# KevinMathewT/multimodal-propaganda-meme-classification

Hardware: AMD Instinct MI355X
Metric: memes/sec (fine-tune step) ViT-B/16+BERT-base bs=32, 1/2/4/8 MI355X (higher is better)
Workload: dtype fp16

## Files before the change

include/memehip.h:

```cpp
#ifndef MEMEHIP_H
#define MEMEHIP_H

#include <stdint.h>

#ifdef __cplusplus
extern "C" {
#endif

typedef enum MhStatus {
    MH_OK = 0,
    MH_EINVAL = 1,
    MH_ESHAPE = 2,
    MH_ELAUNCH = 3
} MhStatus;

typedef void* mh_stream_t;

const char* mh_version(void);
const char* mh_status_str(int status);

#define MH_GEMM_MAX_GROUP 8
#define MH_GEMM_GELU 1
#define MH_GEMM_OUT_F32 2
#define MH_GEMM_ACCUM 4
#define MH_GEMM_QUICK_GELU 8
#define MH_GEMM_DERIV_AUX 16

typedef struct MhGemmProblem {
    const void* A;
    const void* B;
    void* C;
    const float* bias;
    const void* residual;
    void* aux;
    const void* mul;
    float* rowsum;
    int32_t M, N, K;
    int32_t lda, ldb, ldc;
    int32_t flags;
    float alpha;
    const uint32_t* drop_rng;
    float drop_p;
    uint32_t drop_stream;
    const int32_t* rows_dev;
    const int32_t* drop_rows;
    int32_t ksplit;
    int32_t reserved_;
} MhGemmProblem;

int mh_gemm_bf16_grouped(const MhGemmProblem* problems , int n_problems, int a_kmajor,
                         int b_kmajor, mh_stream_t stream);
int mh_gemm_ksplit_for(int K, int want);
int mh_gemm_set_trace(void* device_buffer);

int mh_layernorm_fwd(const void* x , const float* gamma, const float* beta, void* y ,
                     float* y_f32 , float* mean, float* rstd,
                     int rows, int D, float eps, mh_stream_t stream);
int mh_layernorm_bwd(const void* dy , const void* x , const float* gamma,
                     const float* mean, const float* rstd, const void* dx_add ,
                     void* dx , float* part , int n_part, int rows, int D,
                     void* dx_drop ,
                     const uint32_t* rng, float drop_p, uint32_t drop_stream, mh_stream_t stream);
#define MH_LN_MAX_JOBS 4
typedef struct MhLnFwdJob {
    const void* x; const float* gamma; const float* beta; void* y; float* y_f32; float* mean; float* rstd;
    int32_t rows; float eps;
    const int32_t* rows_dev;
} MhLnFwdJob;
typedef struct MhLnBwdJob {
    const void* dy; const void* x; const float* gamma; const float* mean; const float* rstd;
    const void* dx_add; void* dx; float* part; void* dx_drop; const uint32_t* rng;
    int32_t n_part; int32_t rows; float drop_p; uint32_t drop_stream;
    const int32_t* rows_dev;
    const int32_t* drop_rows;
} MhLnBwdJob;
int mh_layernorm_fwd_grouped(const MhLnFwdJob* jobs, int n_jobs, int D, mh_stream_t stream);
int mh_layernorm_bwd_grouped(const MhLnBwdJob* jobs, int n_jobs, int D, mh_stream_t stream);
#define MH_COLSUM_MAX_JOBS 64
typedef struct MhColsumJob {
    const float* part;
    float* out0;
    float* out1;
} MhColsumJob;
int mh_colsum_partials_f32(const MhColsumJob* jobs , int n_jobs, int n_part, int D,
                           float scale, mh_stream_t stream);

int mh_attn_fwd(const void* qkv, const int64_t* key_mask, void* out, float* lse, int B, int S, int H,
                const uint32_t* rng, float drop_p, uint32_t drop_stream, mh_stream_t stream);
int mh_attn_bwd(const void* qkv, const int64_t* key_mask, const void* out, const void* dout,
                const float* lse, float* delta, void* dqkv, int B, int S, int H, const uint32_t* rng,
                float drop_p, uint32_t drop_stream, mh_stream_t stream);
int mh_attn_fwd_packed(const void* qkv, const int64_t* key_mask, void* out, float* lse, const int32_t* cu,
                       const int32_t* row_map, int B, int S, int H, const uint32_t* rng, float drop_p,
                       uint32_t drop_stream, mh_stream_t stream);
int mh_attn_bwd_packed(const void* qkv, const int64_t* key_mask, const void* out, const void* dout,
                       const float* lse, float* delta, void* dqkv, const int32_t* cu, const int32_t* row_map, int B,
                       int S, int H, const uint32_t* rng, float drop_p, uint32_t drop_stream, mh_stream_t stream);

#define MH_ATTN_MAX_GROUP 2
typedef struct MhAttnProblem {
    const void* qkv; const int64_t* key_mask; void* out; float* lse;
    const void* dout; float* delta; void* dqkv;
    const int32_t* cu; const int32_t* row_map;
    const uint32_t* rng; float drop_p; uint32_t drop_stream;
    int32_t B, S, H; int32_t reserved;
} MhAttnProblem;
int mh_attn_fwd_grouped(const MhAttnProblem* problems , int n, mh_stream_t stream);
int mh_attn_bwd_grouped(const MhAttnProblem* problems , int n, mh_stream_t stream);
int mh_attn_set_onepass(int on);

int mh_pack_plan(const int64_t* mask , int B, int S, int pool_index, int32_t* cu, int32_t* row_map,
                 int32_t* inv_map, int64_t* pmask, int32_t* pool_rows, int32_t* n_rows, mh_stream_t stream);
int mh_pack_rows(const void* src , const int32_t* row_map, const int32_t* n_rows, void* dst,
                 int max_rows, int D, mh_stream_t stream);
int mh_unpack_rows(const void* src , const int32_t* inv_map, void* dst ,
                   int max_rows, int D, mh_stream_t stream);

#define MH_ROWS_MAX_JOBS 8
typedef struct {
    const void* src;
    void* dst;
    const int32_t* idx;
    const int32_t* rows_dev;
    int32_t n, rows, D, stride, offset; int32_t reserved_;
} MhRowsJob;
int mh_rows_gather(const MhRowsJob* jobs , int n_jobs, mh_stream_t stream);
int mh_rows_scatter_zero(const MhRowsJob* jobs , int n_jobs, mh_stream_t stream);

int mh_bert_embed_fwd(const int64_t* ids, const float* word, const float* pos, const float* type0,
                      const float* gamma, const float* beta, void* pre ,
                      void* y , float* mean, float* rstd, int B, int S, int D, int vocab,
                      float eps, const uint32_t* rng, float drop_p, uint32_t drop_stream ,
                      mh_stream_t stream);
int mh_bert_embed_bwd(const int64_t* ids, const void* d_pre , float* dword ,
                      float* dpos , float* dtype0 , int B, int S, int D,
// ... 251 lines not shown
```

multimodal_propaganda_meme_classification_amd/_lib.py:

```python
from __future__ import annotations

import ctypes as C
import os

_HERE = os.path.dirname(os.path.abspath(__file__))
LIB_PATH = os.path.join(_HERE, "libmemehip.so")
LIB_PATH_F16 = os.path.join(_HERE, "libmemehip_f16.so")
LIB_PATHS = {"bf16": LIB_PATH, "fp16": LIB_PATH_F16}

MH_GEMM_MAX_GROUP = 8
MH_GEMM_GELU = 1
MH_GEMM_OUT_F32 = 2
MH_GEMM_ACCUM = 4
MH_GEMM_QUICK_GELU = 8
MH_GEMM_DERIV_AUX = 16
MH_COLSUM_MAX_JOBS = 64
MH_LN_MAX_JOBS = 4
MH_ATTN_MAX_GROUP = 2

c_void_p, c_int, c_int64, c_float = C.c_void_p, C.c_int, C.c_int64, C.c_float


class MhGemmProblem(C.Structure):
    _fields_ = [("A", c_void_p), ("B", c_void_p), ("C", c_void_p), ("bias", c_void_p),
# ... 17 lines not shown
    _fields_ = [("slabs", c_void_p), ("g", c_void_p)] + [(n, C.c_int32) for n in ("Cout", "Cin", "KH", "KW", "Cp", "ldk", "nsplit", "accumulate")] + \
               [("scale", C.c_float), ("block_start", C.c_int32)]


class MhConvGeom(C.Structure):
    _fields_ = [(n, C.c_int32) for n in ("B", "H", "W", "C", "KH", "KW", "stride", "pad", "Cout", "ldk")]


class MhConvBnBwd(C.Structure):
    _fields_ = [(n, c_void_p) for n in ("z", "mean", "rstd", "gamma", "beta", "part")] + [("relu", C.c_int32), ("reserved_", C.c_int32),
                                                                                          ("addend", c_void_p), ("y_mask", c_void_p)]


class MhConvWgradProblem(C.Structure):
    _fields_ = [("dy", c_void_p), ("x", c_void_p), ("slabs", c_void_p), ("ksplit", C.c_int32), ("alpha", C.c_float), ("geom", MhConvGeom)]


MH_CONV_MAX_GROUP = 6
MH_CONV_MAX_JOBS = 64
MH_BN_RELU, MH_BN_ACCUM_PARAM_GRADS = 1, 2


MH_ADAM_MAX_GROUPS = 8


class MhAdamSkipGroups(C.Structure):
    _fields_ = [("hyper", c_void_p * MH_ADAM_MAX_GROUPS), ("beta1", C.c_double * MH_ADAM_MAX_GROUPS), ("beta2", C.c_double * MH_ADAM_MAX_GROUPS),
                ("n", C.c_int32), ("reserved_", C.c_int32)]


class MhLossScale(C.Structure):
    _fields_ = [("scale", c_void_p), ("growth", c_void_p), ("overflow", c_void_p), ("growth_factor", C.c_float), ("backoff_factor", C.c_float),
                ("min_scale", C.c_float), ("max_scale", C.c_float), ("growth_interval", C.c_int32), ("base_grad_scale", C.c_float)]


class MhLnFwdJob(C.Structure):
    _fields_ = [(n, c_void_p) for n in ("x", "gamma", "beta", "y", "y_f32", "mean", "rstd")] + \
               [("rows", C.c_int32), ("eps", C.c_float), ("rows_dev", c_void_p)]


class MhLnBwdJob(C.Structure):
    _fields_ = [(n, c_void_p) for n in ("dy", "x", "gamma", "mean", "rstd", "dx_add", "dx", "part", "dx_drop", "rng")] + \
               [("n_part", C.c_int32), ("rows", C.c_int32), ("drop_p", C.c_float), ("drop_stream", C.c_uint32),
                ("rows_dev", c_void_p), ("drop_rows", c_void_p)]


class MhAttnProblem(C.Structure):
    _fields_ = [(n, c_void_p) for n in ("qkv", "key_mask", "out", "lse", "dout", "delta", "dqkv", "cu", "row_map", "rng")] + \
               [("drop_p", C.c_float), ("drop_stream", C.c_uint32), ("B", C.c_int32), ("S", C.c_int32), ("H", C.c_int32),
                ("reserved", C.c_int32)]


MH_ROWS_MAX_JOBS = 8


class MhRowsJob(C.Structure):
    _fields_ = [(n, c_void_p) for n in ("src", "dst", "idx", "rows_dev")] + \
               [(n, C.c_int32) for n in ("n", "rows", "D", "stride", "offset", "reserved_")]


class MhGemmF32(C.Structure):
    _fields_ = [("A", c_void_p), ("B", c_void_p), ("C", c_void_p), ("bias", c_void_p)] + \
               [(n, C.c_int32) for n in ("M", "N", "K", "lda", "ldb", "ldc", "flags")] + \
               [(n, c_void_p) for n in ("bn_gamma", "bn_beta", "bn_running_mean", "bn_running_var", "bn_save_mean",
                                        "bn_save_rstd", "bn_z")] + \
               [("bn_ldz", C.c_int32), ("bn_eps", C.c_float), ("bn_momentum", C.c_float), ("bn_training", C.c_int32)]


MH_F32_ACCUM, MH_F32_TANH, MH_F32_RELU, MH_F32_BN = 1, 2, 4, 8


class MhHeadParams(C.Structure):
    _fields_ = [(n, c_void_p) for n in ("Wt", "bt", "Wi", "bi", "Wf", "bf_", "Wo", "bo")]


class MhHeadGrads(C.Structure):
    _fields_ = [(n, c_void_p) for n in ("Wt", "bt", "Wi", "bi", "Wf", "bf_", "Wo", "bo")]


_PROTOS = {
    "mh_gemm_bf16_grouped": [C.POINTER(MhGemmProblem), c_int, c_int, c_int, c_void_p],
    "mh_gemm_set_trace": [c_void_p],
    "mh_gemm_ksplit_for": [c_int, c_int],
    "mh_layernorm_fwd": [c_void_p] * 7 + [c_int, c_int, c_float, c_void_p],
    "mh_layernorm_bwd": [c_void_p] * 8 + [c_int, c_int, c_int, c_void_p, c_void_p, c_float, C.c_uint32, c_void_p],
    "mh_layernorm_fwd_grouped": [C.POINTER(MhLnFwdJob), c_int, c_int, c_void_p],
    "mh_layernorm_bwd_grouped": [C.POINTER(MhLnBwdJob), c_int, c_int, c_void_p],
    "mh_colsum_partials_f32": [C.POINTER(MhColsumJob), c_int, c_int, c_int, c_float, c_void_p],
    "mh_attn_fwd": [c_void_p] * 4 + [c_int, c_int, c_int, c_void_p, c_float, C.c_uint32, c_void_p],
    "mh_attn_bwd": [c_void_p] * 7 + [c_int, c_int, c_int, c_void_p, c_float, C.c_uint32, c_void_p],
    "mh_attn_fwd_grouped": [C.POINTER(MhAttnProblem), c_int, c_void_p],
    "mh_attn_bwd_grouped": [C.POINTER(MhAttnProblem), c_int, c_void_p],
    "mh_attn_set_onepass": [c_int],
    "mh_attn_fwd_packed": [c_void_p] * 6 + [c_int, c_int, c_int, c_void_p, c_float, C.c_uint32, c_void_p],
    "mh_attn_bwd_packed": [c_void_p] * 9 + [c_int, c_int, c_int, c_void_p, c_float, C.c_uint32, c_void_p],
    "mh_pack_plan": [c_void_p, c_int, c_int, c_int] + [c_void_p] * 6 + [c_void_p],
    "mh_pack_rows": [c_void_p] * 4 + [c_int, c_int, c_void_p],
    "mh_unpack_rows": [c_void_p] * 3 + [c_int, c_int, c_void_p],
    "mh_rows_gather": [C.POINTER(MhRowsJob), c_int, c_void_p],
    "mh_rows_scatter_zero": [C.POINTER(MhRowsJob), c_int, c_void_p],
    "mh_bert_embed_fwd": [c_void_p] * 10 + [c_int, c_int, c_int, c_int, c_float, c_void_p, c_float, C.c_uint32, c_void_p],
    "mh_image_normalize_u8": [c_void_p, c_void_p, c_int, c_int, c_int, C.POINTER(c_float), C.POINTER(c_float), c_void_p],
    "mh_image_resample_u8": [c_void_p] * 5 + [c_int] + [c_void_p] * 2 + [c_int] + [c_void_p] * 4 + [c_int] * 5 + [c_void_p],
    "mh_image_luma_sum_u8": [c_void_p, c_void_p, c_int, c_int, c_void_p],
    "mh_image_jitter_rotate_u8": [c_void_p] * 5 + [c_int] * 3 + [c_void_p],
    "mh_dropout_apply": [c_void_p, c_int64, c_void_p, c_float, C.c_uint32, c_void_p],
    "mh_dropout_mask_u8": [c_void_p, c_int64, c_void_p, c_float, C.c_uint32, c_void_p],
    "mh_bert_embed_bwd": [c_void_p] * 5 + [c_int, c_int, c_int, c_int, c_int64, c_float, c_void_p, c_void_p, c_void_p, c_void_p],
    "mh_position_ids_from_input_ids": [c_void_p] * 3 + [c_int] * 4 + [c_void_p],
    "mh_bert_embed_fwd_pos": [c_void_p] * 10 + [c_int, c_int, c_int, c_int, c_float, c_void_p, c_float, C.c_uint32, c_void_p, c_int,
                              c_void_p],
    "mh_embed_pos_bwd": [c_void_p] * 5 + [c_int] * 4 + [c_float, c_void_p],
    "mh_zero_rows_f32": [c_void_p, c_void_p, c_int, c_int, c_int, c_void_p],
    "mh_patchify": [c_void_p, c_void_p] + [c_int] * 5 + [c_void_p],
    "mh_patchify_ld": [c_void_p, c_void_p] + [c_int] * 6 + [c_void_p],
    "mh_copy2d_u32": [c_void_p, c_int, c_void_p, c_int, c_int, c_int, c_int, c_void_p],
    "mh_vit_assemble_fwd": [c_void_p] * 4 + [c_int] * 3 + [c_void_p],
    "mh_vit_assemble_bwd": [c_void_p] * 4 + [c_int] * 3 + [c_float, c_void_p],
    "mh_head_fwd": [C.POINTER(MhHeadParams), c_void_p, c_void_p, c_int] + [c_void_p] * 4 + [c_int] * 7 + [c_void_p, c_float, C.c_uint32, c_void_p, c_void_p],
    "mh_head_bwd": [C.POINTER(MhHeadParams), C.POINTER(MhHeadGrads)] + [c_void_p] * 8 + [c_int] * 8 + [c_float, c_void_p, c_float, C.c_uint32, c_void_p, c_void_p],
    "mh_pool_fwd": [c_void_p, c_void_p, c_int, c_void_p] + [c_int] * 5 + [c_void_p, c_void_p],
    "mh_pool_bwd": [c_void_p, c_void_p, c_void_p, c_int] + [c_int] * 5 + [c_float, c_void_p, c_void_p],
    "mh_bn1d_fwd": [c_void_p, c_int, c_void_p, c_void_p, c_void_p, c_void_p, c_void_p, c_int, c_void_p, c_void_p, c_int, c_int,
                    c_float, c_float, c_int, c_int, c_void_p],
    "mh_bn1d_bwd": [c_void_p, c_int, c_void_p, c_int, c_void_p, c_int, c_void_p, c_void_p, c_void_p, c_void_p, c_int, c_void_p,
                    c_void_p, c_int, c_int, c_int, c_void_p],
    "mh_gemm_f32": [C.POINTER(MhGemmF32), c_int, c_int, c_void_p],
    "mh_colsum_f32": [c_void_p, c_int, c_void_p, c_int, c_int, c_float, c_void_p],
    "mh_pool_max_fwd": [c_void_p, c_void_p, c_void_p, c_int, c_int, c_int, c_void_p],
    "mh_pool_max_bwd": [c_void_p, c_void_p, c_void_p, c_int, c_int, c_int, c_void_p],
    "mh_pool_mean_fwd": [c_void_p, c_void_p, c_void_p, c_int, c_int, c_int, c_void_p],
    "mh_pool_mean_bwd": [c_void_p, c_void_p, c_void_p, c_int, c_int, c_int, c_void_p],
    "mh_pool_attn_fwd": [c_void_p] * 7 + [c_int] * 4 + [c_void_p],
    "mh_pool_attn_bwd": [c_void_p] * 9 + [c_int] * 4 + [c_void_p],
    "mh_pad_seq_f32": [c_void_p, c_void_p] + [c_int] * 5 + [c_void_p],
    "mh_relu_max_fwd": [c_void_p, c_void_p, c_void_p] + [c_int] * 4 + [c_void_p],
    "mh_relu_max_bwd": [c_void_p, c_void_p, c_void_p] + [c_int] * 3 + [c_void_p],
    "mh_conv_fold_f32": [c_void_p, c_void_p] + [c_int] * 7 + [c_void_p],
    "mh_mca3_fwd": [c_void_p] * 9 + [c_int, c_int, c_void_p],
    "mh_mca3_bwd": [c_void_p] * 15 + [c_int, c_int, c_void_p],
    "mh_softmax_gate_fwd": [c_void_p, c_void_p, c_void_p, c_int, c_int, c_void_p],
    "mh_softmax_gate_bwd": [c_void_p] * 5 + [c_int, c_int, c_void_p],
    "mh_nchw_to_nhwc": [c_void_p, c_void_p] + [c_int] * 5 + [c_void_p],
    "mh_im2col_nhwc": [c_void_p, c_void_p] + [c_int] * 9 + [c_void_p],
    "mh_col2im_nhwc": [c_void_p, c_void_p] + [c_int] * 9 + [c_void_p],
    "mh_conv_weight_pack": [c_void_p, c_void_p] + [c_int] * 6 + [c_void_p],
    "mh_conv_weight_unpack": [c_void_p, c_void_p] + [c_int] * 6 + [c_float, c_void_p],
    "mh_conv_weight_pack_batched": [C.POINTER(MhConvPackJob), c_int, c_void_p],
    "mh_conv_wgrad_finish_batched": [C.POINTER(MhConvWgradJob), c_int, c_void_p],
    "mh_conv_splitk": [C.POINTER(MhConvGeom), c_int],
    "mh_conv_fwd": [c_void_p, c_void_p, c_void_p, c_void_p, c_void_p, C.POINTER(MhConvGeom), c_void_p],
    "mh_conv_dgrad": [c_void_p, c_void_p, c_void_p, c_void_p, C.POINTER(MhConvGeom), C.POINTER(MhConvBnBwd), c_void_p],
    "mh_conv_dgrad_pair": [c_void_p, c_void_p, c_void_p, c_void_p, c_int, c_int, c_void_p, C.POINTER(MhConvGeom), C.POINTER(MhConvBnBwd), c_void_p],
    "mh_bn2d_bwd_parts": [c_void_p, c_void_p, c_void_p, c_int] + [c_void_p] * 7 + [c_int, c_int, c_int, c_float, c_void_p],
    "mh_conv_wgrad": [c_void_p, c_void_p, c_void_p, c_int, c_float, C.POINTER(MhConvGeom), c_void_p],
    "mh_conv_wgrad_grouped": [C.POINTER(MhConvWgradProblem), c_int, c_void_p],
    "mh_bn2d_fwd_parts": [c_void_p, c_void_p, c_int] + [c_void_p] * 8 + [c_int, c_int, c_float, c_float, c_int, c_void_p],
    "mh_bn2d_workspace_elems": [c_int, c_int],
    "mh_bn2d_fwd": [c_void_p] * 10 + [c_int, c_int, c_float, c_float, c_int, c_int, c_void_p],
    "mh_bn2d_apply": [c_void_p] * 7 + [c_int, c_int, c_int, c_void_p],
    "mh_bn2d_bwd": [c_void_p] * 12 + [c_int, c_int, c_int, c_float, c_void_p],
    "mh_maxpool_fwd": [c_void_p, c_void_p, c_void_p] + [c_int] * 7 + [c_void_p],
    "mh_maxpool_bwd": [c_void_p, c_void_p, c_void_p] + [c_int] * 7 + [c_void_p],
    "mh_avgpool_fwd": [c_void_p, c_void_p, c_int, c_int, c_int, c_void_p],
    "mh_avgpool_bwd": [c_void_p, c_void_p, c_int, c_int, c_int, c_float, c_void_p],
    "mh_add_h16": [c_void_p, c_void_p, c_void_p, c_int64, c_void_p],
# ... 69 lines not shown
```

multimodal_propaganda_meme_classification_amd/csrc/gemm.hip:

```cpp
#include "common.h"
#include "gemm_tile.h"
#include <stdlib.h>

namespace {
using namespace mh_tile;


struct DevProblem {
    MhGemmProblem p;
    int tiles_n;
    int tile_start;
    int tiles_m;
    int kchunk;
};
struct GemmGroup {
    int n;
    int total_tiles;
    int group_m;
    int pad_;
    float* sk_partial;
    unsigned* sk_flags;
    unsigned long long* trace;
    const int* rows_any;
    DevProblem d[MH_GEMM_MAX_GROUP];
};
MH_DEV void trace_stamp(const GemmGroup& g, int k) {
    if (g.trace && threadIdx.x == 0) g.trace[(size_t)blockIdx.x * 4 + k] = wall_clock64();
}

template <int TM, int NTHR>
struct EpiPrefetch {
    static constexpr int iters = TM * 16 / NTHR;
    i32x4 res[iters], mul[iters];
};
template <int TM, int NTHR>
MH_DEV void epilogue_prefetch(const MhGemmProblem& P, int m0, int n0, int tid, int M, EpiPrefetch<TM, NTHR>& pf) {
#pragma unroll
    for (int it = 0; it < EpiPrefetch<TM, NTHR>::iters; ++it) {
        const int q = it * NTHR + tid;
        const int row = q >> 4, cc = q & 15;
        const int gm = min(m0 + row, M - 1), gn = min(n0 + cc * 8, P.N - 8);
        const size_t o = (size_t)gm * P.ldc + gn;
        pf.res[it] = i32x4{0, 0, 0, 0};
        pf.mul[it] = i32x4{0, 0, 0, 0};
        if (P.residual) pf.res[it] = *(const i32x4*)((const h16*)P.residual + o);
        if (P.mul) pf.mul[it] = *(const i32x4*)((const h16*)P.mul + o);
    }
}

template <int TM, int NTHR = TM * 2, bool DROP = true, int PREF = 0>
MH_DEV void epilogue_rows(const MhGemmProblem& P, const float* cs, int m0, int n0, int tid, int M,
                          const EpiPrefetch<TM, NTHR>* pf = nullptr, const f32x4* bias_pre = nullptr) {
    const int flags = P.flags;
    const int ldc = P.ldc, N = P.N;
    const float alpha = P.alpha == 0.f ? 1.0f : P.alpha;
    const h16* const p_mul = (const h16*)P.mul;
    const h16* const p_res = (const h16*)P.residual;
    h16* const p_aux = (h16*)P.aux;
    void* const p_c = P.C;
    const int* const drop_rows = P.drop_rows;
    const DropCtx drop = mh_drop_ctx(DROP ? P.drop_rng : nullptr, P.drop_p, P.drop_stream);
    constexpr int nthreads = NTHR;
    constexpr int iters = TM * 16 / NTHR;
    static_assert(NTHR % 16 == 0, "a thread keeps its column block across iterations");
    const int cc = tid & 15, gn = n0 + cc * 8;
    f32x4 b0 = f32x4{0.f, 0.f, 0.f, 0.f}, b1 = b0;
    if (bias_pre) {
        b0 = bias_pre[0];
        b1 = bias_pre[1];
    } else if (P.bias && gn < N) {
        b0 = *(const f32x4*)(P.bias + gn);
        b1 = *(const f32x4*)(P.bias + gn + 4);
    }
    __builtin_amdgcn_s_waitcnt(0x0F70);
#pragma unroll
    for (int it = 0; it < iters; ++it) {
        const int row = (it * nthreads + tid) >> 4;
        const int gm = m0 + row;
        if (gm >= M || gn >= N) continue;
        float v[8];
        {
            const f32x4 x0 = *(const f32x4*)(cs + cs_index(row, cc * 8));
            const f32x4 x1 = *(const f32x4*)(cs + cs_index(row, cc * 8 + 4));
#pragma unroll
            for (int e = 0; e < 4; ++e) { v[e] = x0[e] * alpha + b0[e]; v[4 + e] = x1[e] * alpha + b1[e]; }
        }
        const size_t o = (size_t)gm * ldc + gn;
        if (DROP && drop.on) {
            const uint64_t dr = drop_rows ? (uint64_t)drop_rows[gm] : (uint64_t)gm;
#pragma unroll
            for (int e = 0; e < 8; ++e) v[e] *= mh_drop_mul(drop, dr * (uint64_t)N + (uint64_t)(gn + e));
        }
        if ((flags & MH_GEMM_GELU) && (flags & MH_GEMM_DERIV_AUX) && p_aux) {
            Pack8 u;
            if (flags & MH_GEMM_QUICK_GELU) {
#pragma unroll
                for (int e = 0; e < 8; ++e) {
                    const float sg = qgelu_sig(v[e]);
                    u.e[e] = mh_f2bf(sg * (1.0f + 1.702f * v[e] * (1.0f - sg)));
                    v[e] *= sg;
                }
            } else {
#pragma unroll
                for (int e = 0; e < 8; ++e) {
                    const GeluParts gp = gelu_parts(v[e]);
                    u.e[e] = mh_f2bf(gp.cdf + v[e] * gp.pdf);
                    v[e] *= gp.cdf;
                }
            }
            *(i32x4*)(p_aux + o) = u.v;
        } else {
            if (p_aux) {
                Pack8 u;
#pragma unroll
                for (int e = 0; e < 8; ++e) u.e[e] = mh_f2bf(v[e]);
                *(i32x4*)(p_aux + o) = u.v;
            }
            if (flags & MH_GEMM_GELU) {
                if (flags & MH_GEMM_QUICK_GELU) {
#pragma unroll
                    for (int e = 0; e < 8; ++e) v[e] = qgelu_f(v[e]);
                } else {
#pragma unroll
                    for (int e = 0; e < 8; ++e) v[e] = gelu_f(v[e]);
                }
            }
        }
        if (p_mul) {
            Pack8 u;
            if (PREF == 1) u.v = pf->mul[it];
            else if (PREF == 2 && !p_res) u.v = pf->res[it];
            else u.v = *(const i32x4*)(p_mul + o);
            if (flags & MH_GEMM_DERIV_AUX) {
#pragma unroll
                for (int e = 0; e < 8; ++e) v[e] *= mh_bf2f(u.e[e]);
            } else if (flags & MH_GEMM_QUICK_GELU) {
#pragma unroll
                for (int e = 0; e < 8; ++e) v[e] *= dqgelu_f(mh_bf2f(u.e[e]));
            } else {
#pragma unroll
                for (int e = 0; e < 8; ++e) v[e] *= dgelu_f(mh_bf2f(u.e[e]));
            }
        }
        if (p_res) {
            Pack8 u;
            if (PREF) u.v = pf->res[it];
            else u.v = *(const i32x4*)(p_res + o);
#pragma unroll
            for (int e = 0; e < 8; ++e) v[e] += mh_bf2f(u.e[e]);
        }
        if (flags & MH_GEMM_OUT_F32) {
            float* c = (float*)p_c + o;
            if (flags & MH_GEMM_ACCUM) {
                const f32x4 c0 = *(const f32x4*)c, c1 = *(const f32x4*)(c + 4);
#pragma unroll
                for (int e = 0; e < 4; ++e) { v[e] += c0[e]; v[4 + e] += c1[e]; }
            }
            *(f32x4*)c = f32x4{v[0], v[1], v[2], v[3]};
            *(f32x4*)(c + 4) = f32x4{v[4], v[5], v[6], v[7]};
        } else {
            Pack8 u;
#pragma unroll
            for (int e = 0; e < 8; ++e) u.e[e] = mh_f2bf(v[e]);
            *(i32x4*)((h16*)p_c + o) = u.v;
        }
    }
}


template <int LA, int LB, bool DROP>
__global__ __launch_bounds__(512, 4) void gemm_kernel(const GemmGroup g) {
    extern __shared__ __attribute__((aligned(16))) char smem[];

    trace_stamp(g, 0);
    int cnt[MH_GEMM_MAX_GROUP], tml[MH_GEMM_MAX_GROUP], liv[MH_GEMM_MAX_GROUP];
#pragma unroll
    for (int i = 0; i < MH_GEMM_MAX_GROUP; ++i) liv[i] = 0x7fffffff;
    if (LA == 0 && g.rows_any) {
        int v[MH_GEMM_MAX_GROUP];
#pragma unroll
        for (int i = 0; i < MH_GEMM_MAX_GROUP; ++i) {
            const int* src = (i < g.n && g.d[i].p.rows_dev) ? g.d[i].p.rows_dev : g.rows_any;
            v[i] = *src;
        }
#pragma unroll
        for (int i = 0; i < MH_GEMM_MAX_GROUP; ++i)
            if (i < g.n && g.d[i].p.rows_dev) liv[i] = __builtin_amdgcn_readfirstlane(v[i]);
    }
    int nwg = 0;
#pragma unroll
    for (int i = 0; i < MH_GEMM_MAX_GROUP; ++i) {
        cnt[i] = 0; tml[i] = 0;
        if (i < g.n) {
            tml[i] = g.d[i].tiles_m;
            cnt[i] = (i + 1 < g.n ? g.d[i + 1].tile_start : g.total_tiles) - g.d[i].tile_start;
            if (LA == 0 && g.d[i].p.rows_dev) {
                tml[i] = min(tml[i], (max(liv[i], 0) + BM - 1) / BM);
                cnt[i] = tml[i] * g.d[i].tiles_n;
            }
            nwg += cnt[i];
        }
    }
    int t;
    {
        const int b = blockIdx.x;
        const int q = nwg >> 3, r = nwg & 7, x = b & 7, j = b >> 3;
        if (j >= q + (x < r ? 1 : 0)) return;
        t = (x < r ? x * (q + 1) : r * (q + 1) + (x - r) * q) + j;
    }
    int pi = 0, tstart = 0, tm_live = tml[0], live = liv[0];
    {
        int acc = 0;
#pragma unroll
        for (int i = 1; i < MH_GEMM_MAX_GROUP; ++i) {
            acc += cnt[i - 1];
            if (i < g.n && t >= acc) { pi = i; tstart = acc; tm_live = tml[i]; live = liv[i]; }
        }
    }
    const MhGemmProblem& P = g.d[pi].p;
    int lt = t - tstart;
    const int kchunk = g.d[pi].kchunk;
    int ksplit_idx = 0;
    if (kchunk > 0) {
        const int per = g.d[pi].tiles_m * g.d[pi].tiles_n;
        ksplit_idx = lt / per;
        lt -= ksplit_idx * per;
    }
    int tm, tn;
    tile_coords(g.d[pi].tiles_n, tm_live, g.group_m, lt, tm, tn);
    const int m0 = tm * BM, n0 = tn * BN;

    int M = P.M, K = P.K;
    const int N = P.N;
    if (P.rows_dev) {
        if (LA == 0) {
            M = min(M, live);
            if (m0 >= M) return;
        } else {
            K = min(K, __builtin_amdgcn_readfirstlane(*P.rows_dev));
        }
    }
    const int kbeg = ksplit_idx * kchunk;
    const int kend = kchunk > 0 ? min(K, kbeg + kchunk) : K;
    const int tid = threadIdx.x, lane = tid & 63, wave = tid >> 6;

    const uint32_t a_bytes = (LA == 0) ? (uint32_t)((M - 1) * P.lda + K) * 2u
                                       : (uint32_t)((K - 1) * P.lda + M) * 2u;
    const uint32_t b_bytes = (LB == 0) ? (uint32_t)((N - 1) * P.ldb + K) * 2u
                                       : (uint32_t)((K - 1) * P.ldb + N) * 2u;
    const __amdgpu_buffer_rsrc_t ra = mh_rsrc(P.A, a_bytes);
    const __amdgpu_buffer_rsrc_t rb = mh_rsrc(P.B, b_bytes);

    f32x4 accb[NI];
#pragma unroll
    for (int i = 0; i < NI; ++i) accb[i] = f32x4{0.f, 0.f, 0.f, 0.f};
    const bool do_rowsum = (LA == 1) && (P.rowsum != nullptr) && (tn == 0) && ((wave % NWN) == 0);
    h16x8 ones;
#pragma unroll
    for (int j = 0; j < 8; ++j) ones[j] = (h16)1.0f;

    const int nk = kend > kbeg ? (kend - kbeg + BK - 1) / BK : 0;
    f32x4 acc[NI][NJ];
    k_loop<LA, LB>(
        acc, smem, nk, wave, lane,
        [&](int kt, char* st) {
            dma_tile<LA, 16 / NW>(ra, P.lda, m0, kbeg + kt * BK, wave, lane, st);
            dma_tile<LB, 16 / NW>(rb, P.ldb, n0, kbeg + kt * BK, wave, lane, st + BM * BK * 2);
        },
        [&](const h16x8 (&fa)[NI]) {
            if (do_rowsum) {
#pragma unroll
                for (int i = 0; i < NI; ++i) accb[i] = MH_MFMA_16x16x32(fa[i], ones, accb[i], 0, 0, 0);
            }
        },
        [&] { trace_stamp(g, 1); });

    trace_stamp(g, 2);
    if (do_rowsum && (lane & 15) == 0) {
#pragma unroll
        for (int i = 0; i < NI; ++i)
#pragma unroll
            for (int r = 0; r < 4; ++r) {
                const int row = m0 + wave_m0(wave) + i * 16 + (lane >> 4) * 4 + r;
                if (row < M) P.rowsum[row] = accb[i][r] * (P.alpha == 0.f ? 1.0f : P.alpha);
            }
    }
    float* cs = (float*)smem;
    if (kchunk > 0) {
        stage_acc(cs, acc, wave, lane);
        __syncthreads();
        float* slab = (float*)P.C + (size_t)ksplit_idx * (size_t)P.M * (size_t)P.ldc;
        store_slab(slab, cs, P.alpha == 0.f ? 1.0f : P.alpha, m0, n0, M, N, P.ldc, tid);
        trace_stamp(g, 3);
        return;
    }
    EpiPrefetch<BM, NW * 64> pf;
    epilogue_prefetch<BM, NW * 64>(P, m0, n0, tid, M, pf);
    stage_acc(cs, acc, wave, lane);
    __syncthreads();
    epilogue_rows<BM, NW * 64, DROP, 1>(P, cs, m0, n0, tid, M, &pf);
    trace_stamp(g, 3);
}

unsigned long long* g_trace = nullptr;

#ifdef MH_LAB
#include "lab/gemm_lab.inc"
#endif

template <int LA, int LB, bool DROP>
int launch2(const GemmGroup& g, hipStream_t s) {
    static bool attr_set = false;
    if (!attr_set) {
        (void)hipFuncSetAttribute((const void*)gemm_kernel<LA, LB, DROP>, hipFuncAttributeMaxDynamicSharedMemorySize, LDS_BYTES);
        attr_set = true;
    }
    hipLaunchKernelGGL((gemm_kernel<LA, LB, DROP>), dim3(g.total_tiles), dim3(512), LDS_BYTES, s, g);
    return mh_launch_status();
}
template <int LA, int LB>
int launch(const GemmGroup& g, hipStream_t s) {
    bool any_drop = false;
    for (int i = 0; i < g.n; ++i) any_drop |= (g.d[i].p.drop_rng != nullptr && g.d[i].p.drop_p > 0.f);
    if (LA == 0 && LB == 0 && any_drop) return launch2<LA, LB, true>(g, s);
    return launch2<LA, LB, false>(g, s);
}

}

extern "C" int mh_gemm_bf16_grouped(const MhGemmProblem* problems, int n_problems, int a_kmajor,
                                    int b_kmajor, mh_stream_t stream) {
    if (!problems || n_problems < 1 || n_problems > MH_GEMM_MAX_GROUP) return MH_EINVAL;
#ifdef MH_LAB
    if (g_variant < 0) {
        const char* e = getenv("MEMEHIP_GEMM_VARIANT");
        g_variant = e ? atoi(e) : -2;
        if (g_variant < 0 || g_variant > 13) g_variant = -2;
    }
    if (g_variant >= 0) {
        const int rc = lab_gemm_grouped(problems, n_problems, a_kmajor, b_kmajor, stream);
        if (rc != LAB_NOT_MINE) return rc;
    }
#endif
    GemmGroup g;
    g.n = n_problems;
    int total = 0;
    for (int i = 0; i < n_problems; ++i) {
        const MhGemmProblem& p = problems[i];
        if (!p.A || !p.B || !p.C) return MH_EINVAL;
        if (p.M < 1 || p.N < 1 || p.K < 1) return MH_ESHAPE;
        if (p.N % 8) return MH_ESHAPE;
        if (a_kmajor && (p.M % 8)) return MH_ESHAPE;
        if (!(a_kmajor && b_kmajor) && (p.K % BK)) return MH_ESHAPE;
        if ((p.lda % 8) || (p.ldb % 8) || (p.ldc % 8)) return MH_ESHAPE;
        if (((uintptr_t)p.A | (uintptr_t)p.B | (uintptr_t)p.C) & 15) return MH_EINVAL;
        if (p.rowsum && !a_kmajor) return MH_EINVAL;
        if ((p.flags & MH_GEMM_ACCUM) && !(p.flags & MH_GEMM_OUT_F32)) return MH_EINVAL;
        g.d[i].p = p;
        g.d[i].tiles_n = (p.N + BN - 1) / BN;
        g.d[i].tile_start = total;
        g.d[i].tiles_m = (p.M + BM - 1) / BM;
        g.d[i].kchunk = 0;
        int splits = 1;
        if (p.ksplit > 1) {
            if (!(p.flags & MH_GEMM_OUT_F32) || (p.flags & (MH_GEMM_ACCUM | MH_GEMM_GELU)) || p.bias || p.residual || p.aux || p.mul ||
                p.rowsum || p.rows_dev || p.drop_rng)
                return MH_EINVAL;
            const int kc = ksplit_chunk(p.K, p.ksplit);
            g.d[i].kchunk = kc;
            splits = (p.K + kc - 1) / kc;
            if (splits != p.ksplit) return MH_ESHAPE;
        }
        total += g.d[i].tiles_m * g.d[i].tiles_n * splits;
    }
    g.total_tiles = total;
    g.group_m = group_m_setting();
    g.pad_ = 0;
    g.trace = g_trace;
    g.sk_partial = nullptr;
    g.sk_flags = nullptr;
    g.rows_any = nullptr;
    for (int i = 0; i < n_problems; ++i)
        if (problems[i].rows_dev && !g.rows_any) g.rows_any = problems[i].rows_dev;
    hipStream_t s = (hipStream_t)stream;
    if (!a_kmajor && !b_kmajor) return launch<0, 0>(g, s);
    if (!a_kmajor && b_kmajor) return launch<0, 1>(g, s);
    if (a_kmajor && b_kmajor) return launch<1, 1>(g, s);
    return MH_EINVAL;
}

extern "C" int mh_gemm_ksplit_for(int K, int want) { return ksplit_fit(K, want); }

extern "C" int mh_gemm_set_trace(void* device_buffer) {
    g_trace = (unsigned long long*)device_buffer;
    return MH_OK;
}

#ifdef MH_LAB
extern "C" int64_t mh_gemm_streamk_workspace_bytes(void) { return (int64_t)(SK_GRID * SK_PARTIAL_FLOATS * 4 + (SK_GRID + 16) * 4); }
extern "C" int mh_gemm_set_streamk(void* workspace, int mode) {
    if (mode < 0 || mode > 2 || (mode > 0 && !workspace)) return MH_EINVAL;
    g_sk_partial = (float*)workspace;
    g_sk_flags = workspace ? (unsigned*)((char*)workspace + SK_GRID * SK_PARTIAL_FLOATS * 4) : nullptr;
    g_sk_mode = workspace ? mode : 0;
    g_sk_force = mode == 2;
    return MH_OK;
}
extern "C" int mh_gemm_set_variant(int v) {
    if (v != -2 && (v < 0 || v > 13)) return MH_EINVAL;
    g_variant = v;
    return MH_OK;
}
#endif
```

Before: 3411.

## Add skinny-M GEMM kernel with deep register prefetch for small-M problems

Adds a dedicated single-wave GEMM kernel for problems with M ≤ 64 and no row indirection, split-K or dropout. It tiles only along N in 16-column strips and keeps a deep ring of register-prefetched K tiles, so small GEMMs (such as head or pooled layers) spread across many workgroups instead of a few large 512-thread tiles that waste most rows. The shared epilogue is factored into reusable helpers. The risk is lower MFMA efficiency per wave and the cost of re-reading A once per N-strip.

```diff
diff --git a/include/memehip.h b/include/memehip.h
--- a/include/memehip.h
+++ b/include/memehip.h
@@ -51,6 +51,7 @@
 int mh_gemm_bf16_grouped(const MhGemmProblem* problems , int n_problems, int a_kmajor,
                          int b_kmajor, mh_stream_t stream);
 int mh_gemm_ksplit_for(int K, int want);
+int mh_gemm_skinny_eligible(const MhGemmProblem* problems , int n_problems, int a_kmajor, int b_kmajor);
 int mh_gemm_set_trace(void* device_buffer);
 
 int mh_layernorm_fwd(const void* x , const float* gamma, const float* beta, void* y ,
diff --git a/multimodal_propaganda_meme_classification_amd/_lib.py b/multimodal_propaganda_meme_classification_amd/_lib.py
--- a/multimodal_propaganda_meme_classification_amd/_lib.py
+++ b/multimodal_propaganda_meme_classification_amd/_lib.py
@@ -123,6 +123,7 @@
     "mh_gemm_bf16_grouped": [C.POINTER(MhGemmProblem), c_int, c_int, c_int, c_void_p],
     "mh_gemm_set_trace": [c_void_p],
     "mh_gemm_ksplit_for": [c_int, c_int],
+    "mh_gemm_skinny_eligible": [C.POINTER(MhGemmProblem), c_int, c_int, c_int],
     "mh_layernorm_fwd": [c_void_p] * 7 + [c_int, c_int, c_float, c_void_p],
     "mh_layernorm_bwd": [c_void_p] * 8 + [c_int, c_int, c_int, c_void_p, c_void_p, c_float, C.c_uint32, c_void_p],
     "mh_layernorm_fwd_grouped": [C.POINTER(MhLnFwdJob), c_int, c_int, c_void_p],
diff --git a/multimodal_propaganda_meme_classification_amd/csrc/gemm.hip b/multimodal_propaganda_meme_classification_amd/csrc/gemm.hip
--- a/multimodal_propaganda_meme_classification_amd/csrc/gemm.hip
+++ b/multimodal_propaganda_meme_classification_amd/csrc/gemm.hip
@@ -48,18 +48,120 @@
     }
 }
 
+struct EpiCtx {
+    int flags, ldc, N;
+    float alpha;
+    const h16* p_mul;
+    const h16* p_res;
+    h16* p_aux;
+    void* p_c;
+};
+MH_DEV EpiCtx epi_ctx(const MhGemmProblem& P) {
+    EpiCtx E;
+    E.flags = P.flags;
+    E.ldc = P.ldc;
+    E.N = P.N;
+    E.alpha = P.alpha == 0.f ? 1.0f : P.alpha;
+    E.p_mul = (const h16*)P.mul;
+    E.p_res = (const h16*)P.residual;
+    E.p_aux = (h16*)P.aux;
+    E.p_c = P.C;
+    return E;
+}
+MH_DEV void epilogue_acc8(const EpiCtx& E, const f32x4 x0, const f32x4 x1, const f32x4 b0, const f32x4 b1, float (&v)[8]) {
+    const float alpha = E.alpha;
+#pragma unroll
+    for (int e = 0; e < 4; ++e) { v[e] = x0[e] * alpha + b0[e]; v[4 + e] = x1[e] * alpha + b1[e]; }
+}
+template <int PREF>
+MH_DEV void epilogue_elem8(const EpiCtx& E, float (&v)[8], int gm, int gn, const i32x4 pf_mul, const i32x4 pf_res) {
+    const int flags = E.flags;
+    const h16* const p_mul = E.p_mul;
+    const h16* const p_res = E.p_res;
+    h16* const p_aux = E.p_aux;
+    const size_t o = (size_t)gm * E.ldc + gn;
+    if ((flags & MH_GEMM_GELU) && (flags & MH_GEMM_DERIV_AUX) && p_aux) {
+        Pack8 u;
+        if (flags & MH_GEMM_QUICK_GELU) {
+#pragma unroll
+            for (int e = 0; e < 8; ++e) {
+                const float sg = qgelu_sig(v[e]);
+                u.e[e] = mh_f2bf(sg * (1.0f + 1.702f * v[e] * (1.0f - sg)));
+                v[e] *= sg;
+            }
+        } else {
+#pragma unroll
+            for (int e = 0; e < 8; ++e) {
+                const GeluParts gp = gelu_parts(v[e]);
+                u.e[e] = mh_f2bf(gp.cdf + v[e] * gp.pdf);
+                v[e] *= gp.cdf;
+            }
+        }
+        *(i32x4*)(p_aux + o) = u.v;
+    } else {
+        if (p_aux) {
+            Pack8 u;
+#pragma unroll
+            for (int e = 0; e < 8; ++e) u.e[e] = mh_f2bf(v[e]);
+            *(i32x4*)(p_aux + o) = u.v;
+        }
+        if (flags & MH_GEMM_GELU) {
+            if (flags & MH_GEMM_QUICK_GELU) {
+#pragma unroll
+                for (int e = 0; e < 8; ++e) v[e] = qgelu_f(v[e]);
+            } else {
+#pragma unroll
+                for (int e = 0; e < 8; ++e) v[e] = gelu_f(v[e]);
+            }
+        }
+    }
+    if (p_mul) {
+        Pack8 u;
+        if (PREF == 1) u.v = pf_mul;
+        else if (PREF == 2 && !p_res) u.v = pf_res;
+        else u.v = *(const i32x4*)(p_mul + o);
+        if (flags & MH_GEMM_DERIV_AUX) {
+#pragma unroll
+            for (int e = 0; e < 8; ++e) v[e] *= mh_bf2f(u.e[e]);
+        } else if (flags & MH_GEMM_QUICK_GELU) {
+#pragma unroll
+            for (int e = 0; e < 8; ++e) v[e] *= dqgelu_f(mh_bf2f(u.e[e]));
+        } else {
+#pragma unroll
+            for (int e = 0; e < 8; ++e) v[e] *= dgelu_f(mh_bf2f(u.e[e]));
+        }
+    }
+    if (p_res) {
+        Pack8 u;
+        if (PREF) u.v = pf_res;
+        else u.v = *(const i32x4*)(p_res + o);
+#pragma unroll
+        for (int e = 0; e < 8; ++e) v[e] += mh_bf2f(u.e[e]);
+    }
+    if (flags & MH_GEMM_OUT_F32) {
+        float* c = (float*)E.p_c + o;
+        if (flags & MH_GEMM_ACCUM) {
+            const f32x4 c0 = *(const f32x4*)c, c1 = *(const f32x4*)(c + 4);
+#pragma unroll
+            for (int e = 0; e < 4; ++e) { v[e] += c0[e]; v[4 + e] += c1[e]; }
+        }
+        *(f32x4*)c = f32x4{v[0], v[1], v[2], v[3]};
+        *(f32x4*)(c + 4) = f32x4{v[4], v[5], v[6], v[7]};
+    } else {
+        Pack8 u;
+#pragma unroll
+        for (int e = 0; e < 8; ++e) u.e[e] = mh_f2bf(v[e]);
+        *(i32x4*)((h16*)E.p_c + o) = u.v;
+    }
+}
+
 template <int TM, int NTHR = TM * 2, bool DROP = true, int PREF = 0>
 MH_DEV void epilogue_rows(const MhGemmProblem& P, const float* cs, int m0, int n0, int tid, int M,
                           const EpiPrefetch<TM, NTHR>* pf = nullptr, const f32x4* bias_pre = nullptr) {
-    const int flags = P.flags;
-    const int ldc = P.ldc, N = P.N;
-    const float alpha = P.alpha == 0.f ? 1.0f : P.alpha;
-    const h16* const p_mul = (const h16*)P.mul;
-    const h16* const p_res = (const h16*)P.residual;
-    h16* const p_aux = (h16*)P.aux;
-    void* const p_c = P.C;
+    const EpiCtx E = epi_ctx(P);
     const int* const drop_rows = P.drop_rows;
     const DropCtx drop = mh_drop_ctx(DROP ? P.drop_rng : nullptr, P.drop_p, P.drop_stream);
+    const int N = E.N;
     constexpr int nthreads = NTHR;
     constexpr int iters = TM * 16 / NTHR;
     static_assert(NTHR % 16 == 0, "a thread keeps its column block across iterations");
@@ -78,92 +180,17 @@
         const int row = (it * nthreads + tid) >> 4;
         const int gm = m0 + row;
         if (gm >= M || gn >= N) continue;
+        const f32x4 x0 = *(const f32x4*)(cs + cs_index(row, cc * 8));
+        const f32x4 x1 = *(const f32x4*)(cs + cs_index(row, cc * 8 + 4));
         float v[8];
-        {
-            const f32x4 x0 = *(const f32x4*)(cs + cs_index(row, cc * 8));
-            const f32x4 x1 = *(const f32x4*)(cs + cs_index(row, cc * 8 + 4));
-#pragma unroll
-            for (int e = 0; e < 4; ++e) { v[e] = x0[e] * alpha + b0[e]; v[4 + e] = x1[e] * alpha + b1[e]; }
-        }
-        const size_t o = (size_t)gm * ldc + gn;
+        epilogue_acc8(E, x0, x1, b0, b1, v);
         if (DROP && drop.on) {
             const uint64_t dr = drop_rows ? (uint64_t)drop_rows[gm] : (uint64_t)gm;
 #pragma unroll
             for (int e = 0; e < 8; ++e) v[e] *= mh_drop_mul(drop, dr * (uint64_t)N + (uint64_t)(gn + e));
         }
-        if ((flags & MH_GEMM_GELU) && (flags & MH_GEMM_DERIV_AUX) && p_aux) {
-            Pack8 u;
-            if (flags & MH_GEMM_QUICK_GELU) {
-#pragma unroll
-                for (int e = 0; e < 8; ++e) {
-                    const float sg = qgelu_sig(v[e]);
-                    u.e[e] = mh_f2bf(sg * (1.0f + 1.702f * v[e] * (1.0f - sg)));
-                    v[e] *= sg;
-                }
-            } else {
-#pragma unroll
-                for (int e = 0; e < 8; ++e) {
-                    const GeluParts gp = gelu_parts(v[e]);
-                    u.e[e] = mh_f2bf(gp.cdf + v[e] * gp.pdf);
-                    v[e] *= gp.cdf;
-                }
-            }
-            *(i32x4*)(p_aux + o) = u.v;
-        } else {
-            if (p_aux) {
-                Pack8 u;
-#pragma unroll
-                for (int e = 0; e < 8; ++e) u.e[e] = mh_f2bf(v[e]);
-                *(i32x4*)(p_aux + o) = u.v;
-            }
-            if (flags & MH_GEMM_GELU) {
-                if (flags & MH_GEMM_QUICK_GELU) {
-#pragma unroll
-                    for (int e = 0; e < 8; ++e) v[e] = qgelu_f(v[e]);
-                } else {
-#pragma unroll
-                    for (int e = 0; e < 8; ++e) v[e] = gelu_f(v[e]);
-                }
-            }
-        }
-        if (p_mul) {
-            Pack8 u;
-            if (PREF == 1) u.v = pf->mul[it];
-            else if (PREF == 2 && !p_res) u.v = pf->res[it];
-            else u.v = *(const i32x4*)(p_mul + o);
-            if (flags & MH_GEMM_DERIV_AUX) {
-#pragma unroll
-                for (int e = 0; e < 8; ++e) v[e] *= mh_bf2f(u.e[e]);
-            } else if (flags & MH_GEMM_QUICK_GELU) {
-#pragma unroll
-                for (int e = 0; e < 8; ++e) v[e] *= dqgelu_f(mh_bf2f(u.e[e]));
-            } else {
-#pragma unroll
-                for (int e = 0; e < 8; ++e) v[e] *= dgelu_f(mh_bf2f(u.e[e]));
-            }
-        }
-        if (p_res) {
-            Pack8 u;
-            if (PREF) u.v = pf->res[it];
-            else u.v = *(const i32x4*)(p_res + o);
-#pragma unroll
-            for (int e = 0; e < 8; ++e) v[e] += mh_bf2f(u.e[e]);
-        }
-        if (flags & MH_GEMM_OUT_F32) {
-            float* c = (float*)p_c + o;
-            if (flags & MH_GEMM_ACCUM) {
-                const f32x4 c0 = *(const f32x4*)c, c1 = *(const f32x4*)(c + 4);
-#pragma unroll
-                for (int e = 0; e < 4; ++e) { v[e] += c0[e]; v[4 + e] += c1[e]; }
-            }
-            *(f32x4*)c = f32x4{v[0], v[1], v[2], v[3]};
-            *(f32x4*)(c + 4) = f32x4{v[4], v[5], v[6], v[7]};
-        } else {
-            Pack8 u;
-#pragma unroll
-            for (int e = 0; e < 8; ++e) u.e[e] = mh_f2bf(v[e]);
-            *(i32x4*)((h16*)p_c + o) = u.v;
-        }
+        const i32x4 z = i32x4{0, 0, 0, 0};
+        epilogue_elem8<PREF>(E, v, gm, gn, PREF == 1 ? pf->mul[it] : z, PREF ? pf->res[it] : z);
     }
 }
 
@@ -300,6 +327,184 @@
     __syncthreads();
     epilogue_rows<BM, NW * 64, DROP, 1>(P, cs, m0, n0, tid, M, &pf);
     trace_stamp(g, 3);
+}
+
+constexpr int SKN_NJ = 1;
+constexpr int SKN_BN = 16 * SKN_NJ;
+constexpr int SKN_MAX_M = 64;
+constexpr int SKN_CS_LD = SKN_BN + 4;
+constexpr uint32_t SKN_PAST_END = 0x80000000u;
+constexpr int skn_depth(int mi) { return mi <= 2 ? 8 : 4; }
+
+template <int MI>
+struct SknFrag {
+    i32x4 a[MI][2], b[SKN_NJ * 2];
+};
+
+template <int LB, int MI>
+__global__ __launch_bounds__(64) void gemm_skinny_kernel(const GemmGroup g) {
+    constexpr int D = skn_depth(MI), NJ = SKN_NJ, CPR = 2 * NJ;
+    constexpr int CS_FLOATS = MI * 16 * SKN_CS_LD, IMG_FLOATS = BK * SKN_BN * 2 / 4;
+    __shared__ __attribute__((aligned(16))) float cs[CS_FLOATS > IMG_FLOATS ? CS_FLOATS : IMG_FLOATS];
+    int t;
+    {
+        const int nwg = g.total_tiles, b = blockIdx.x;
+        const int q = nwg >> 3, r = nwg & 7, x = b & 7, j = b >> 3;
+        if (j >= q + (x < r ? 1 : 0)) return;
+        t = (x < r ? x * (q + 1) : r * (q + 1) + (x - r) * q) + j;
+    }
+    int pi = 0;
+#pragma unroll
+    for (int i = 1; i < MH_GEMM_MAX_GROUP; ++i)
+        if (i < g.n && t >= g.d[i].tile_start) pi = i;
+    const MhGemmProblem& P = g.d[pi].p;
+    const int n0 = (t - g.d[pi].tile_start) * SKN_BN;
+    const int M = P.M, N = P.N, K = P.K, lda = P.lda, ldb = P.ldb;
+    const int lane = threadIdx.x, r16 = lane & 15, g4 = lane >> 4;
+    const __amdgpu_buffer_rsrc_t ra = mh_rsrc(P.A, (uint32_t)((M - 1) * lda + K) * 2u);
+    const __amdgpu_buffer_rsrc_t rb = mh_rsrc(P.B, LB == 0 ? (uint32_t)((N - 1) * ldb + K) * 2u : (uint32_t)((K - 1) * ldb + N) * 2u);
+    const int nk = K / BK;
+
+    const uint32_t a_off = (uint32_t)(r16 * lda + g4 * 8) * 2u, a_blk = (uint32_t)(16 * lda) * 2u;
+    const uint32_t b_off = LB == 0 ? (uint32_t)((n0 + r16) * ldb + g4 * 8) * 2u : (uint32_t)((lane / CPR) * ldb + n0 + (lane % CPR) * 8) * 2u;
+    const uint32_t b_blk = (uint32_t)(16 * ldb) * 2u;
+    const uint32_t b_piece = (uint32_t)((64 / CPR) * ldb) * 2u;
+    const uint32_t b_tile = LB == 0 ? (uint32_t)BK * 2u : (uint32_t)(BK * ldb) * 2u;
+    auto load = [&](SknFrag<MI>& f, int kt) {
+        const bool in = kt < nk;
+        const uint32_t ao = in ? a_off + (uint32_t)kt * (BK * 2u) : SKN_PAST_END;
+        const uint32_t bo = in ? b_off + (uint32_t)kt * b_tile : SKN_PAST_END;
+#pragma unroll
+        for (int p = 0; p < CPR; ++p) f.b[p] = mh_buf_load16(rb, LB == 0 ? bo + (p >> 1) * b_blk + (p & 1) * 64u : bo + p * b_piece);
+#pragma unroll
+        for (int i = 0; i < MI; ++i)
+#pragma unroll
+            for (int h = 0; h < 2; ++h) f.a[i][h] = mh_buf_load16(ra, ao + i * a_blk + h * 64u);
+    };
+
+    f32x4 acc[MI][NJ];
+#pragma unroll
+    for (int i = 0; i < MI; ++i)
+#pragma unroll
+        for (int j = 0; j < NJ; ++j) acc[i][j] = f32x4{0.f, 0.f, 0.f, 0.f};
+    SknFrag<MI> ring[D];
+#pragma unroll
+    for (int s = 0; s < D; ++s) load(ring[s], s);
+    char* const wimg = (char*)cs;
+    auto consume = [&](const SknFrag<MI>& f) {
+        Pack8 fb[NJ][2];
+        if (LB == 0) {
+#pragma unroll
+            for (int p = 0; p < CPR; ++p) fb[p >> 1][p & 1].v = f.b[p];
+        } else {
+            asm volatile("" ::: "memory");
+#pragma unroll
+            for (int p = 0; p < CPR; ++p) *(i32x4*)(wimg + p * 1024 + lane * 16) = f.b[p];
+            asm volatile("" ::: "memory");
+#pragma unroll
+            for (int j = 0; j < NJ; ++j)
+#pragma unroll
+                for (int kk = 0; kk < 2; ++kk) {
+                    const int k0 = kk * 32 + g4 * 8 + (r16 >> 2);
+                    const int at = k0 * (SKN_BN * 2) + j * 32 + (r16 & 3) * 8;
+                    union {
+                        struct { s16x4 lo, hi; } s;
+                        h16x8 h;
+                    } cv;
+                    cv.s.lo = __builtin_amdgcn_ds_read_tr16_b64_v4i16(LDS_PTR(s16x4, wimg + at));
+                    cv.s.hi = __builtin_amdgcn_ds_read_tr16_b64_v4i16(LDS_PTR(s16x4, wimg + at + 4 * (SKN_BN * 2)));
+                    fb[j][kk].h = cv.h;
+                }
+            asm volatile("" ::: "memory");
+        }
+#pragma unroll
+        for (int kk = 0; kk < 2; ++kk)
+#pragma unroll
+            for (int i = 0; i < MI; ++i) {
+                Pack8 fa;
+                fa.v = f.a[i][kk];
+#pragma unroll
+                for (int j = 0; j < NJ; ++j) acc[i][j] = MH_MFMA_16x16x32(fa.h, fb[j][kk].h, acc[i][j], 0, 0, 0);
+            }
+    };
+    int kt0 = 0;
+    for (; kt0 + D <= nk; kt0 += D) {
+#pragma unroll
+        for (int s = 0; s < D; ++s) {
+            consume(ring[s]);
+            load(ring[s], kt0 + s + D);
+        }
+    }
+    const int rem = nk - kt0;
+#pragma unroll
+    for (int s = 0; s < D - 1; ++s)
+        if (s < rem) consume(ring[s]);
+
+    const EpiCtx E = epi_ctx(P);
+    constexpr int iters = MI * 16 * CPR / 64, RPI = 64 / CPR;
+    const int cc = lane % CPR, gn = n0 + cc * 8;
+    f32x4 b0 = f32x4{0.f, 0.f, 0.f, 0.f}, b1 = b0;
+    if (P.bias && gn < N) {
+        b0 = *(const f32x4*)(P.bias + gn);
+        b1 = *(const f32x4*)(P.bias + gn + 4);
+    }
+    i32x4 pf_mul[iters], pf_res[iters];
+#pragma unroll
+    for (int it = 0; it < iters; ++it) {
+        const size_t o = (size_t)min(it * RPI + lane / CPR, M - 1) * E.ldc + min(gn, N - 8);
+        pf_mul[it] = pf_res[it] = i32x4{0, 0, 0, 0};
+        if (E.p_res) pf_res[it] = *(const i32x4*)(E.p_res + o);
+        if (E.p_mul) pf_mul[it] = *(const i32x4*)(E.p_mul + o);
+    }
+    asm volatile("" ::: "memory");
+#pragma unroll
+    for (int i = 0; i < MI; ++i)
+#pragma unroll
+        for (int j = 0; j < NJ; ++j)
+#pragma unroll
+            for (int r = 0; r < 4; ++r) cs[(i * 16 + g4 * 4 + r) * SKN_CS_LD + j * 16 + r16] = acc[i][j][r];
+    asm volatile("" ::: "memory");
+#pragma unroll
+    for (int it = 0; it < iters; ++it) {
+        const int gm = it * RPI + lane / CPR;
+        if (gm >= M || gn >= N) continue;
+        const f32x4 x0 = *(const f32x4*)(cs + gm * SKN_CS_LD + cc * 8);
+        const f32x4 x1 = *(const f32x4*)(cs + gm * SKN_CS_LD + cc * 8 + 4);
+        float v[8];
+        epilogue_acc8(E, x0, x1, b0, b1, v);
+        epilogue_elem8<1>(E, v, gm, gn, pf_mul[it], pf_res[it]);
+    }
+}
+
+constexpr int SKN_WIDE_TILES = 128;
+bool skinny_eligible(const MhGemmProblem* problems, int n, int a_kmajor, int b_kmajor) {
+    if (!problems || n < 1 || n > MH_GEMM_MAX_GROUP || a_kmajor) return false;
+    int wide_tiles = 0;
+    for (int i = 0; i < n; ++i) {
+        const MhGemmProblem& p = problems[i];
+        if (p.M < 1 || p.M > SKN_MAX_M || p.rows_dev || p.ksplit > 1 || p.drop_rng) return false;
+        wide_tiles += (p.N + BN - 1) / BN;
+    }
+    return wide_tiles < SKN_WIDE_TILES;
+}
+
+template <int LB, int MI>
+int launch_skinny2(const GemmGroup& g, hipStream_t s) {
+    hipLaunchKernelGGL((gemm_skinny_kernel<LB, MI>), dim3(g.total_tiles), dim3(64), 0, s, g);
+    return mh_launch_status();
+}
+int launch_skinny(GemmGroup& g, int b_kmajor, hipStream_t s) {
+    int total = 0, max_m = 0;
+    for (int i = 0; i < g.n; ++i) {
+        g.d[i].tiles_n = (g.d[i].p.N + SKN_BN - 1) / SKN_BN;
+        g.d[i].tiles_m = 1;
+        g.d[i].tile_start = total;
+        total += g.d[i].tiles_n;
+        max_m = g.d[i].p.M > max_m ? g.d[i].p.M : max_m;
+    }
+    g.total_tiles = total;
+    if (max_m <= 32) return b_kmajor ? launch_skinny2<1, 2>(g, s) : launch_skinny2<0, 2>(g, s);
+    return b_kmajor ? launch_skinny2<1, 4>(g, s) : launch_skinny2<0, 4>(g, s);
 }
 
 unsigned long long* g_trace = nullptr;
@@ -383,6 +588,7 @@
     for (int i = 0; i < n_problems; ++i)
         if (problems[i].rows_dev && !g.rows_any) g.rows_any = problems[i].rows_dev;
     hipStream_t s = (hipStream_t)stream;
+    if (skinny_eligible(problems, n_problems, a_kmajor, b_kmajor)) return launch_skinny(g, b_kmajor, s);
     if (!a_kmajor && !b_kmajor) return launch<0, 0>(g, s);
     if (!a_kmajor && b_kmajor) return launch<0, 1>(g, s);
     if (a_kmajor && b_kmajor) return launch<1, 1>(g, s);
@@ -390,6 +596,10 @@
 }
 
 extern "C" int mh_gemm_ksplit_for(int K, int want) { return ksplit_fit(K, want); }
+
+extern "C" int mh_gemm_skinny_eligible(const MhGemmProblem* problems, int n_problems, int a_kmajor, int b_kmajor) {
+    return skinny_eligible(problems, n_problems, a_kmajor, b_kmajor) ? 1 : 0;
+}
 
 extern "C" int mh_gemm_set_trace(void* device_buffer) {
     g_trace = (unsigned long long*)device_buffer;
```

New measurement: 3449, median of 6. 1.1% higher.
